# genjax-dev/genjax

Measured on AMD Instinct MI355X. Metric: particles/sec (particle-steps/s), bootstrap SMC sweep, linear-Gaussian SSM T=100, higher is better.
Workload: dtype f32; 1 GPU; BASELINE config 2: linear-Gaussian state-space (T=100), bootstrap SMC, systematic resampling every step; particles_per_gpu=1000000, particles_total=1000000, T=100, resampler=systematic, graph=True, key=314159

## Files before the change

### genjax_amd/_lib.py

```python
from __future__ import annotations

import ctypes
import os
from ctypes import (POINTER, Structure, c_char_p, c_float, c_int, c_int32, c_int64,
                    c_size_t, c_uint32, c_uint64, c_void_p)

import torch

GMX_MAX_IN = 64
GMX_MAX_OUT = 64
GMX_MAX_TAB = 8
GMX_MAX_UNI = 64

ABI_VERSION = 8
ANC_TAG_SHIFT = 24
ANC_INDEX_MASK = (1 << ANC_TAG_SHIFT) - 1
ANC_TAG_MAX = 255
KEY_NONE, KEY_ARRAY, KEY_SPLIT, KEY_ROWSPLIT, KEY_BCAST = 0, 1, 2, 3, 4
RESAMPLE_SYSTEMATIC, RESAMPLE_STRATIFIED, RESAMPLE_MULTINOMIAL, RESAMPLE_MULTINOMIAL_TILED = 0, 1, 2, 3
RESAMPLE_MULTINOMIAL_SORTED = 4


class ResampleIn(Structure):
    _fields_ = [
# ... 54 lines not shown
    _fields_ = [
        ("in_d", c_void_p * GMX_MAX_IN),
        ("out_d", c_void_p * GMX_MAX_OUT),
        ("tab_d", c_void_p * GMX_MAX_TAB),
        ("uni", c_uint32 * GMX_MAX_UNI),
        ("ancestors_d", c_void_p),
        ("key_mode", c_int32),
        ("key0", c_uint32),
        ("key1", c_uint32),
        ("keys_d", c_void_p),
        ("key_inner", c_int64),
        ("index_offset", c_int64),
        ("red_out_d", c_void_p),
        ("tile_agg_d", c_void_p),
        ("tile_shift", c_int32),
        ("reserved_", c_int32),
        ("step_stride", c_int64),
        ("rs", ResampleIn),
        ("sh", ShardIn),
        ("peer", Peer),
    ]


class GenmiError(RuntimeError):
    pass


_LIB_DIR = os.path.join(os.path.dirname(os.path.abspath(__file__)), "lib")
LIB_PATH = os.environ.get("GENMI_LIB") or os.path.join(_LIB_DIR, "libgenmi_hip.so")


class Backend:

    def __init__(self, cdll, device: torch.device, uses_streams: bool):
        self.c = cdll
        self.device = device
        self.uses_streams = uses_streams
        self._proto()

    def _proto(self):
        c = self.c
        c.gmx_run_args_bytes.restype = c_size_t
        if int(c.gmx_run_args_bytes()) != ctypes.sizeof(RunArgs):
            raise GenmiError(f"gmx_run_args is {c.gmx_run_args_bytes()} bytes in the library and {ctypes.sizeof(RunArgs)} in "
                             "this binding (genjax_amd/_lib.py): rebuild both from one include/genmi.h")
        c.gmx_version.restype = c_int
        c.gmx_last_error.restype = c_char_p
        c.gmx_threefry2x32_host.argtypes = [c_uint32, c_uint32, c_uint32, c_uint32, POINTER(c_uint32)]
        c.gmx_threefry2x32_host.restype = None
        c.gmx_split.argtypes = [POINTER(c_uint32), c_int64, c_int64, c_void_p, c_void_p]
        c.gmx_split_rows.argtypes = [c_void_p, c_int64, c_int64, c_void_p, c_void_p]
        c.gmx_fold_in.argtypes = [c_void_p, c_uint32, c_int64, c_void_p, c_void_p]
        c.gmx_random_bits.argtypes = [c_void_p, c_int64, c_int64, c_void_p, c_void_p]
        c.gmx_program_create.argtypes = [POINTER(c_uint32), c_size_t, POINTER(c_void_p)]
        c.gmx_program_destroy.argtypes = [c_void_p]
        c.gmx_program_specialize.argtypes = [c_void_p]
        c.gmx_program_is_specialized.argtypes = [c_void_p]
        c.gmx_program_code_hash.argtypes = [c_void_p]
        c.gmx_program_code_hash.restype = c_uint64
        c.gmx_program_despecialize.argtypes = [c_void_p, ctypes.c_char_p]
        c.gmx_jit_rejected_count.argtypes = []
        c.gmx_jit_rejected_count.restype = c_int64
        c.gmx_program_grid.argtypes = [c_void_p, c_int64]
        c.gmx_program_grid.restype = c_int64
        c.gmx_program_run.argtypes = [c_void_p, c_int64, POINTER(RunArgs), c_void_p]
        c.gmx_program_writes_tile_stats.argtypes = [c_void_p]
        c.gmx_program_set_background.argtypes = [c_void_p, c_uint32]
        c.gmx_program_set_fuse_resample.argtypes = [c_void_p]
        c.gmx_program_set_fuse_resample_loop.argtypes = [c_void_p]
        c.gmx_program_fuses_resample.argtypes = [c_void_p]
        c.gmx_program_set_fuse_shard_step.argtypes = [c_void_p]
        c.gmx_program_fuses_shard_step.argtypes = [c_void_p]
        c.gmx_program_resident_particles.argtypes = [c_void_p]
        c.gmx_program_resident_particles.restype = c_int64
        c.gmx_logsumexp_workspace.argtypes = [c_int64, c_int64]
        c.gmx_logsumexp_workspace.restype = c_size_t
        c.gmx_logsumexp.argtypes = [c_void_p, c_int64, c_int64, c_void_p, c_void_p, c_void_p, c_void_p]
        c.gmx_sum_rows_inorder.argtypes = [c_void_p, c_int64, c_int64, c_int64, c_int64, c_void_p, c_void_p]
        c.gmx_sum_rows_workspace.argtypes = [c_int64, c_int64]
        c.gmx_sum_rows_workspace.restype = c_size_t
        c.gmx_sum_rows.argtypes = [c_void_p, c_int64, c_int64, c_void_p, c_void_p, c_void_p]
        c.gmx_reduce_max.argtypes = [c_void_p, c_int64, c_void_p, c_void_p]
        c.gmx_weight_cdf_workspace.argtypes = [c_int64]
        c.gmx_weight_cdf_workspace.restype = c_size_t
        c.gmx_weight_cdf.argtypes = [c_void_p, c_int64, c_int, c_void_p, c_int64, c_void_p, c_void_p,
                                     c_void_p, c_void_p, c_void_p]
        c.gmx_ancestors.argtypes = [c_int, POINTER(c_uint32), c_void_p, c_int64, c_uint64, c_void_p,
                                    c_int64, c_int64, c_int64, c_void_p, c_void_p]
        c.gmx_multinomial_workspace.argtypes = [c_int64]
        c.gmx_multinomial_workspace.restype = c_size_t
        c.gmx_multinomial.argtypes = [POINTER(c_uint32), c_void_p, c_int64, c_void_p, c_int64, c_void_p, c_void_p, c_void_p]
        c.gmx_resample_workspace.argtypes = [c_int64]
        c.gmx_resample_workspace.restype = c_size_t
        c.gmx_resample.argtypes = [c_int, POINTER(c_uint32), c_void_p, c_int64, c_int, c_void_p, c_int64, c_void_p,
                                   c_void_p, c_void_p, c_void_p, c_void_p]
        c.gmx_tile_stats.argtypes = [c_void_p, c_int64, c_int, c_void_p, c_void_p, c_void_p]
        c.gmx_resample_tiles.argtypes = [c_int, POINTER(c_uint32), c_void_p, c_int64, c_int, c_void_p, c_void_p, c_void_p,
                                         c_void_p, c_void_p, c_void_p]
        c.gmx_multinomial_tiled_workspace.argtypes = [c_int64]
        c.gmx_multinomial_tiled_workspace.restype = c_size_t
        c.gmx_multinomial_tiled.argtypes = [POINTER(c_uint32), c_void_p, c_int64, c_int, c_void_p, c_void_p, c_void_p,
                                            c_void_p, c_void_p, c_void_p, c_void_p, c_int, c_void_p]
        c.gmx_slot_uniforms.argtypes = [c_void_p, c_int, c_int64, c_void_p, c_int, c_void_p]
        c.gmx_resample_tiles_u.argtypes = [c_int, POINTER(c_uint32), c_void_p, c_int64, c_int, c_void_p, c_void_p, c_void_p,
                                           c_void_p, c_void_p, c_void_p, c_void_p]
        c.gmx_sorted_uniforms_words.argtypes = [c_int64]
# ... 135 lines not shown
```

### genjax_amd/csrc/gmx_kernels.hip

```cpp
#include <hip/hip_runtime.h>
#include <hip/hiprtc.h>
#include <stdio.h>
#include <stdlib.h>
#include <string.h>
#include <sys/stat.h>
#include <unistd.h>

#include <new>
#include <atomic>
#include <string>
#include <vector>

#include "gmx_block.h"
#include "gmx_vm.h"
#include "gmx_resample.h"
#include "gmx_peer.h"
#include "gmx_sorted.h"
#include "gmx_offspring.h"
#include "gmx_shard_fill.h"

#define GMX_HIP(call)                                                        \
  do {                                                                       \
    hipError_t _e = (call);                                                  \
    if (_e != hipSuccess) return gmx_fail("%s (hip error %lld)", hipGetErrorString(_e), (long long)_e); \
// ... 756 lines not shown
  gmx_key k; k.k0 = kk.x; k.k1 = kk.y;
  gmx_key o = gmx_fold_in(k, data);
  reinterpret_cast<uint2*>(out)[i] = make_uint2(o.k0, o.k1);
}
__global__ void __launch_bounds__(GMX_BLOCK)
k_random_bits(const uint32_t* __restrict__ keys, int64_t n, int64_t m, uint32_t* __restrict__ out) {
  int64_t t = (int64_t)blockIdx.x * GMX_BLOCK + threadIdx.x;
  if (t >= n * m) return;
  int64_t i = t / m, j = t - i * m;
  uint2 kk = reinterpret_cast<const uint2*>(keys)[i];
  gmx_key k; k.k0 = kk.x; k.k1 = kk.y;
  out[t] = gmx_bits32(k, (uint64_t)j);
}

static inline dim3 grid_for(int64_t n) { return dim3((unsigned)((n + GMX_BLOCK - 1) / GMX_BLOCK)); }

extern "C" int gmx_split(const uint32_t key[2], int64_t n, int64_t index_offset,
                         uint32_t* out_keys_d, gmx_stream stream) {
  if (!key || (n > 0 && !out_keys_d)) return gmx_fail("gmx_split: null argument%s");
  if (n <= 0) return 0;
  hipLaunchKernelGGL(k_split, grid_for(n), dim3(GMX_BLOCK), 0, (hipStream_t)stream, key[0], key[1],
                     n, index_offset, out_keys_d);
  GMX_HIP(hipGetLastError());
  return 0;
}
extern "C" int gmx_split_rows(const uint32_t* keys_d, int64_t rows, int64_t inner,
                              uint32_t* out_keys_d, gmx_stream stream) {
  if (rows <= 0 || inner <= 0) return 0;
  if (!keys_d || !out_keys_d) return gmx_fail("gmx_split_rows: null argument%s");
  hipLaunchKernelGGL(k_split_rows, grid_for(rows * inner), dim3(GMX_BLOCK), 0, (hipStream_t)stream,
                     keys_d, rows, inner, out_keys_d);
  GMX_HIP(hipGetLastError());
  return 0;
}
extern "C" int gmx_fold_in(const uint32_t* keys_d, uint32_t data, int64_t n, uint32_t* out_d,
                           gmx_stream stream) {
  if (n <= 0) return 0;
  if (!keys_d || !out_d) return gmx_fail("gmx_fold_in: null argument%s");
  hipLaunchKernelGGL(k_fold_in, grid_for(n), dim3(GMX_BLOCK), 0, (hipStream_t)stream, keys_d, data, n,
                     out_d);
  GMX_HIP(hipGetLastError());
  return 0;
}
extern "C" int gmx_random_bits(const uint32_t* keys_d, int64_t n, int64_t m, uint32_t* out_d,
                               gmx_stream stream) {
  if (n <= 0 || m <= 0) return 0;
  if (!keys_d || !out_d) return gmx_fail("gmx_random_bits: null argument%s");
  hipLaunchKernelGGL(k_random_bits, grid_for(n * m), dim3(GMX_BLOCK), 0, (hipStream_t)stream, keys_d,
                     n, m, out_d);
  GMX_HIP(hipGetLastError());
  return 0;
}

#define LSE_ITEMS 16
#define LSE_TILE (GMX_BLOCK * LSE_ITEMS)
static_assert(LSE_TILE == GMX_LSE_TILE, "the row reductions' workspaces (gmx_sizes.h) are per tile of LSE_TILE columns");

__device__ __forceinline__ bool lse_finite(float m) { return m > -gmx_inf() && m < gmx_inf(); }
__device__ __forceinline__ float lse_nan_only(float x) { return x != x ? x : 0.0f; }

__global__ void __launch_bounds__(GMX_BLOCK)
k_lse_tiles(const float* __restrict__ lw, int64_t cols, int64_t tiles_per_row,
            float* __restrict__ partials) {
  __shared__ float lds4[4];
  int64_t row = blockIdx.y, tile = blockIdx.x;
  const float* x = lw + row * cols;
  int64_t base = tile * LSE_TILE;
  float v[LSE_ITEMS];
  float m = -gmx_inf();
#pragma unroll
  for (int k = 0; k < LSE_ITEMS; ++k) {
    int64_t j = base + (int64_t)k * GMX_BLOCK + threadIdx.x;
    v[k] = (j < cols) ? x[j] : -gmx_inf();
    m = gmx_rmax(m, v[k]);
  }
  m = block_max(m, lds4);
  float s = 0.0f;
  if (lse_finite(m)) {
#pragma unroll
    for (int k = 0; k < LSE_ITEMS; ++k) s += gmx_expf(v[k] - m);
  } else {
#pragma unroll
    for (int k = 0; k < LSE_ITEMS; ++k) s += lse_nan_only(v[k]);
  }
  s = block_sum(s, lds4);
  if (threadIdx.x == 0) {
    float* p = partials + 2 * (row * tiles_per_row + tile);
    p[0] = m; p[1] = s;
  }
}
__global__ void __launch_bounds__(GMX_BLOCK)
k_lse_final(const float* __restrict__ partials, int64_t n_part, float* __restrict__ out,
            float* __restrict__ out_max) {
  __shared__ float lds4[4];
  int64_t row = blockIdx.x;
  const float* p = partials + 2 * row * n_part;
  float m = -gmx_inf();
  for (int64_t j = threadIdx.x; j < n_part; j += GMX_BLOCK) m = gmx_rmax(m, p[2 * j]);
  m = block_max(m, lds4);
  float s = 0.0f;
  if (lse_finite(m))
    for (int64_t j = threadIdx.x; j < n_part; j += GMX_BLOCK)
      s += p[2 * j + 1] * gmx_expf(p[2 * j] - m);
  else
    for (int64_t j = threadIdx.x; j < n_part; j += GMX_BLOCK) s += lse_nan_only(p[2 * j + 1]);
  s = block_sum(s, lds4);
// ... 2630 lines not shown
```

### genjax_amd/csrc/gmx_math.h

```cpp
#pragma once
#if !defined(__HIPCC_RTC__)
#include <stdint.h>
#else
#include "genmi.h"
#endif

#if defined(__HIPCC__)
#define GMX_HD __host__ __device__ __forceinline__
#define GMX_HDM __host__ __device__ __forceinline__
#else
#define GMX_HD static inline
#define GMX_HDM inline
#endif

#define GMX_INF_BITS 0x7f800000u
#define GMX_NAN_BITS 0x7fc00000u

GMX_HD float gmx_u2f(uint32_t u) {
  union { uint32_t u; float f; } c; c.u = u; return c.f;
}
GMX_HD uint32_t gmx_f2u(float f) {
  union { uint32_t u; float f; } c; c.f = f; return c.u;
}
GMX_HD float gmx_fma(float a, float b, float c) { return __builtin_fmaf(a, b, c); }
// ... 57 lines not shown
  return nan ? x : y;
}

GMX_HD float gmx_expf_nonpos(float x) {
  const float lo = -87.33654022216797f;
  float xc = x < lo ? lo : x;
  float kf = __builtin_rintf(xc * 1.44269502162933349609375f);
  float r = gmx_fma(kf, -0.693359375f, xc);
  r = gmx_fma(kf, 2.12194440e-4f, r);
  float p = 1.9875691500e-4f;
  p = gmx_fma(p, r, 1.3981999507e-3f);
  p = gmx_fma(p, r, 8.3334519073e-3f);
  p = gmx_fma(p, r, 4.1665795894e-2f);
  p = gmx_fma(p, r, 1.6666665459e-1f);
  p = gmx_fma(p, r, 5.0000001201e-1f);
  float r2 = r * r;
  p = gmx_fma(p, r2, r);
  p = p + 1.0f;
  int k = gmx_isnan(x) ? 0 : (int)kf;
  int k1 = k >> 1;
  int k2 = k - k1;
  float y = (p * gmx_pow2i(k1)) * gmx_pow2i(k2);
  y = y < 1.17549435e-38f ? 0.0f : y;
  return x < lo ? 0.0f : y;
}

GMX_HD uint32_t gmx_exp_fixed_packed(float d, int shift) {
  const float lo = -87.33654022216797f;
  float dc = d > lo ? d : lo;
  dc = dc < 100.0f ? dc : 100.0f;
  const float kf = __builtin_rintf(dc * 1.44269502162933349609375f);
  float r = gmx_fma(kf, -0.693359375f, dc);
  r = gmx_fma(kf, 2.12194440e-4f, r);
  float p = 1.9875691500e-4f;
  p = gmx_fma(p, r, 1.3981999507e-3f);
  p = gmx_fma(p, r, 8.3334519073e-3f);
  p = gmx_fma(p, r, 4.1665795894e-2f);
  p = gmx_fma(p, r, 1.6666665459e-1f);
  p = gmx_fma(p, r, 5.0000001201e-1f);
  const float r2 = r * r;
  p = gmx_fma(p, r2, r);
  p = p + 1.0f;
  const uint32_t pb = gmx_f2u(p);
  uint32_t m = (pb & 0x007fffffu) | 0x00800000u;
  int32_t amt = 189 - (int32_t)(pb >> 23) - (int32_t)kf - shift;
  m = amt < 0 ? 0u : m;
  amt = amt > 63 ? 63 : amt;
  amt = amt < 0 ? 0 : amt;
  return m | ((uint32_t)amt << 24);
}
GMX_HD uint64_t gmx_fixed_unpack(uint32_t pk) { return ((uint64_t)(pk & 0x00ffffffu) << 39) >> (pk >> 24); }
GMX_HD uint64_t gmx_exp_fixed(float d, int shift) { return gmx_fixed_unpack(gmx_exp_fixed_packed(d, shift)); }

GMX_HD float gmx_logf(float x) {
  const uint32_t ux = gmx_f2u(x);
  const int den = ux < 0x00800000u;
  const float xs = den ? x * 8388608.0f : x;
  const uint32_t us = gmx_f2u(xs);
  int e = (den ? -23 : 0) + (int)(us >> 23) - 126;
  const float m = gmx_u2f((us & 0x007fffffu) | 0x3f000000u);
  const int low = m < 0.707106781186547524f;
  e -= low;
  const float f = low ? (m + m) - 1.0f : m - 1.0f;
  float z = f * f;
  float p = 7.0376836292e-2f;
  p = gmx_fma(p, f, -1.1514610310e-1f);
  p = gmx_fma(p, f, 1.1676998740e-1f);
  p = gmx_fma(p, f, -1.2420140846e-1f);
  p = gmx_fma(p, f, 1.4249322787e-1f);
  p = gmx_fma(p, f, -1.6668057665e-1f);
  p = gmx_fma(p, f, 2.0000714765e-1f);
  p = gmx_fma(p, f, -2.4999993993e-1f);
  p = gmx_fma(p, f, 3.3333331174e-1f);
  float y = (p * f) * z;
  float ef = (float)e;
  y = gmx_fma(ef, -2.12194440e-4f, y);
  y = gmx_fma(-0.5f, z, y);
  float r = f + y;
  r = gmx_fma(ef, 0.693359375f, r);
  r = (ux == GMX_INF_BITS) ? x : r;
  r = (ux >> 31) ? gmx_nan() : r;
  r = (ux == 0u || ux == 0x80000000u) ? -gmx_inf() : r;
  return gmx_isnan(x) ? x : r;
}

GMX_HD float gmx_log1pf(float x) {
  float u = 1.0f + x;
  float l = gmx_logf(u);
  float d = u - 1.0f;
  float r = l * (x / d);
  r = (gmx_f2u(u) == GMX_INF_BITS) ? u : r;
  r = (u == 1.0f) ? x : r;
  return gmx_isnan(x) ? x : r;
}

GMX_HD float gmx_sqrtf(float x) { return __builtin_sqrtf(x); }

GMX_HD float gmx_softplusf(float x) {
  float ax = gmx_fabs(x);
  float t = gmx_log1pf(gmx_expf(-ax));
  return (x > 0.0f ? x : 0.0f) + t;
}

GMX_HD float gmx_sigmoidf(float x) {
  if (x >= 0.0f) {
    float e = gmx_expf(-x);
    return 1.0f / (1.0f + e);
  }
  float e = gmx_expf(x);
  return e / (1.0f + e);
}

GMX_HD float gmx_tanhf(float x) {
  float ax = gmx_fabs(x);
  if (ax < 1e-4f) return x;
  float e = gmx_expf(-2.0f * ax);
  float t = (1.0f - e) / (1.0f + e);
  return (gmx_f2u(x) >> 31) ? -t : t;
}

GMX_HD float gmx_neg_log1m_sq(float x) {
  const float t = -(x * x);
  const float u = 1.0f + t;
  const uint32_t us = gmx_f2u(u);
  int e = (int)(us >> 23) - 126;
  const float m = gmx_u2f((us & 0x007fffffu) | 0x3f000000u);
  const int low = m < 0.707106781186547524f;
  e -= low;
  const float f = low ? (m + m) - 1.0f : m - 1.0f;
  float z = f * f;
  float p = 7.0376836292e-2f;
  p = gmx_fma(p, f, -1.1514610310e-1f);
  p = gmx_fma(p, f, 1.1676998740e-1f);
  p = gmx_fma(p, f, -1.2420140846e-1f);
  p = gmx_fma(p, f, 1.4249322787e-1f);
  p = gmx_fma(p, f, -1.6668057665e-1f);
  p = gmx_fma(p, f, 2.0000714765e-1f);
  p = gmx_fma(p, f, -2.4999993993e-1f);
  p = gmx_fma(p, f, 3.3333331174e-1f);
  float y = (p * f) * z;
  float ef = (float)e;
  y = gmx_fma(ef, -2.12194440e-4f, y);
  y = gmx_fma(-0.5f, z, y);
  float l = f + y;
  l = gmx_fma(ef, 0.693359375f, l);
  l = (us == 0u) ? -gmx_inf() : l;
  const float d = u - 1.0f;
  float r = l * (t / d);
  r = (u == 1.0f) ? t : r;
  return -r;
}

GMX_HD float gmx_erfinv_central(float w) {
  w = w - 2.5f;
  float p = 2.81022636e-08f;
  p = gmx_fma(p, w, 3.43273939e-07f);
  p = gmx_fma(p, w, -3.5233877e-06f);
  p = gmx_fma(p, w, -4.39150654e-06f);
  p = gmx_fma(p, w, 0.00021858087f);
  p = gmx_fma(p, w, -0.00125372503f);
  p = gmx_fma(p, w, -0.00417768164f);
  p = gmx_fma(p, w, 0.246640727f);
  p = gmx_fma(p, w, 1.50140941f);
  return p;
}
GMX_HD float gmx_erfinv_tail(float w) {
  w = gmx_sqrtf(w) - 3.0f;
  float p = -0.000200214257f;
  p = gmx_fma(p, w, 0.000100950558f);
  p = gmx_fma(p, w, 0.00134934322f);
  p = gmx_fma(p, w, -0.00367342844f);
  p = gmx_fma(p, w, 0.00573950773f);
  p = gmx_fma(p, w, -0.0076224613f);
  p = gmx_fma(p, w, 0.00943887047f);
  p = gmx_fma(p, w, 1.00167406f);
  p = gmx_fma(p, w, 2.83297682f);
  return p;
}
GMX_HD float gmx_erfinvf_from_w(float x, float w) {
  float p;
  if (w < 5.0f) p = gmx_erfinv_central(w);
  else p = gmx_erfinv_tail(w);
  if (gmx_fabs(x) == 1.0f) return x * gmx_inf();
  return p * x;
}
GMX_HD float gmx_erfinvf(float x) { return gmx_erfinvf_from_w(x, -gmx_log1pf(-(x * x))); }
GMX_HD float gmx_erfinvf_unit(float x) { return gmx_erfinvf_from_w(x, gmx_neg_log1m_sq(x)); }

GMX_HD float gmx_lgammaf(float x) {
  if (gmx_isnan(x)) return x;
  if (x <= 0.0f) return gmx_inf();
  if (gmx_f2u(x) == GMX_INF_BITS) return x;
  float shift = 0.0f;
  if (x < 8.0f) {
    float prod = 1.0f;
    while (x < 8.0f) {
      prod = prod * x;
      x = x + 1.0f;
    }
    shift = gmx_logf(prod);
  }
// ... 63 lines not shown
```

### genjax_amd/csrc/gmx_offspring.h

```cpp
#pragma once
#include "gmx_block.h"
#include "gmx_resample.h"
#include "gmx_sorted.h"

#define CDF_VEC_OT 4
#ifndef RS_THREADS
#define RS_THREADS 256
#endif
#define RS_TILE (RS_THREADS * CDF_VEC_OT)
#define RS_MAX_TILES GMX_MAX_TILES
static_assert(RS_TILE == GMX_TILE && RS_THREADS == GMX_BLOCK, "resampling tiles are the CDF's definition tiles");
static_assert(RS_MAX_TILES % GMX_BLOCK == 0, "tile table shape");

#define GMX_ANC_TAG_SHIFT 24
#define GMX_ANC_INDEX_MASK 0xffffffu
#define GMX_ANC_TAG_MAX 255u
__device__ __forceinline__ void gmx_store_u32x4_sc1(uint32_t* p, uint32_t a, uint32_t b, uint32_t c, uint32_t d) {
  typedef uint32_t v4 __attribute__((ext_vector_type(4)));
  v4 v; v.x = a; v.y = b; v.z = c; v.w = d;
  asm volatile("s_nop 1\n\tglobal_store_dwordx4 %0, %1, off sc1\n\ts_nop 1" :: "v"(p), "v"(v) : "memory");
}
__device__ __forceinline__ void gmx_store_u32x8_sc1(uint32_t* base_uniform, uint32_t off, uint4 a, uint4 b) {
  typedef uint32_t v4 __attribute__((ext_vector_type(4)));
  v4 va, vb; va.x = a.x; va.y = a.y; va.z = a.z; va.w = a.w; vb.x = b.x; vb.y = b.y; vb.z = b.z; vb.w = b.w;
// ... 4 lines not shown
  __hip_atomic_store(p, a, __ATOMIC_RELAXED, __HIP_MEMORY_SCOPE_AGENT);
}

typedef uint32_t rs_u32x4_a4 __attribute__((ext_vector_type(4), aligned(4)));
typedef uint32_t sorted_u32x2_a4 __attribute__((ext_vector_type(2), aligned(4)));
struct sorted_ctx {
  const uint32_t* slow; const uint32_t* guide; const uint64_t* toff;
  uint64_t stot, gmax; uint32_t sh, mask; double ratio;
};
__device__ __forceinline__ sorted_ctx sorted_ctx_of(const uint32_t* table, int64_t n, uint64_t total, uint64_t stot, uint32_t sh) {
  const gmx_sorted_layout L = gmx_sorted_layout_of(n);
  sorted_ctx X;
  X.slow = table; X.guide = table + L.off_guide;
  X.toff = reinterpret_cast<const uint64_t*>(table + L.off_toff);
  X.stot = stot;
  X.sh = sh;
  X.mask = (1u << X.sh) - 1u;
  X.gmax = X.stot >> X.sh;
  X.ratio = (double)X.stot / (double)(total ? total : 1ull);
  return X;
}
__device__ __forceinline__ int64_t sorted_below_exact(const sorted_ctx& X, uint64_t c, uint64_t total, int64_t j, int64_t n) {
  const u128 R = mul64(c, X.stot);
  j = j < 0 ? 0 : (j > n ? n : j);
  auto below = [&](int64_t k) {
    const uint64_t off = X.toff[k >> 10];
    const uint64_t S = off + (uint64_t)(uint32_t)(X.slow[k] - (uint32_t)off);
    return gt128(R, mul64(S, total));
  };
  while (j > 0 && !below(j - 1)) --j;
  while (j < n && below(j)) ++j;
  return j;
}

#define RS_TPB 1
#define GMX_KEEP_BRANCH asm volatile("")
__device__ __forceinline__ uint64_t rs_zext_here(uint32_t o) { asm volatile("" : "+v"(o)); return (uint64_t)o; }
#define RS_BLOCK (GMX_BLOCK * RS_TPB)
#define RS_WAVES (RS_BLOCK / GMX_WAVE)
static_assert(RS_MAX_TILES % RS_BLOCK == 0, "tile table shape");
#define RS_FILL_SLOTS 2048
template <int kind, int PER, bool TAGGED>
__device__ __forceinline__ void
gmx_offspring_tile_body(uint32_t k0, uint32_t k1, uint32_t u0_host, const float* __restrict__ lw,
                        const float* __restrict__ tmax, const uint64_t* __restrict__ agg, int64_t n, int n_tiles, float scale,
                        float* __restrict__ max_out, uint64_t* __restrict__ total_out, int32_t* __restrict__ anc,
                        const uint32_t* __restrict__ uslot, uint32_t tag,
                        int tile0 = -1, uint64_t a_prefix = 0ull, uint64_t a_total = 0ull, uint64_t a_mk = 0ull) {
  const int blk = tile0 >= 0 ? tile0 : (int)blockIdx.x;
  const uint32_t tagw = TAGGED ? (tag << GMX_ANC_TAG_SHIFT) : 0u;
  __shared__ uint64_t s_below[RS_WAVES], s_all[RS_WAVES], s_scan[RS_WAVES], s_g[RS_TPB];
  __shared__ float s_max[RS_WAVES];
  const int lane = threadIdx.x & 63, wave = threadIdx.x >> 6;
  const int grp = RS_TPB > 1 ? (int)(threadIdx.x >> 8) : 0, ltid = threadIdx.x & (GMX_BLOCK - 1);
  const int first_tile = blk * RS_TPB;
  const int my_tile = first_tile + grp;
  const bool tile_ok = my_tile < n_tiles;
  const int tile_c = tile_ok ? my_tile : n_tiles - 1;
  const int64_t i0 = (int64_t)tile_c * RS_TILE + (int64_t)ltid * CDF_VEC_OT;
  float x[CDF_VEC_OT];
  const bool full_tile = (int64_t)(tile_c + 1) * RS_TILE <= n;
  if (full_tile) {
    float4 v = *reinterpret_cast<const float4*>(lw + i0);
    x[0] = v.x; x[1] = v.y; x[2] = v.z; x[3] = v.w;
  } else {
#pragma unroll
    for (int c = 0; c < CDF_VEC_OT; ++c) {
      const int64_t ic = i0 + c < n ? i0 + c : n - 1;
      const float xv = lw[ic];
      x[c] = (i0 + c < n) ? xv : -gmx_inf();
    }
  }
  constexpr bool PREF = (PER == 0);
  constexpr int PERN = PREF ? 1 : PER;
  static_assert(PER >= 0 && PER * RS_BLOCK <= RS_MAX_TILES, "rows of the tile table per thread");
  static_assert(!PREF || RS_TPB == 1, "the prefix form works on one tile per block");
  uint64_t ta[PERN];
  float tm[PERN];
  const uint32_t tid4 = threadIdx.x * 4u;
  uint64_t pf_prefix = 0, pf_total = 0, pf_mk = 0;
  if (PREF) {
    if (agg) { pf_prefix = agg[tile_c]; pf_total = agg[n_tiles]; pf_mk = agg[n_tiles + 1]; }
    else { pf_prefix = a_prefix; pf_total = a_total; pf_mk = a_mk; }
  } else {
#pragma unroll
    for (int r = 0; r < PERN; ++r) {
      ta[r] = 0ull; tm[r] = -gmx_inf();
      if (r * RS_BLOCK < n_tiles) {
        if ((r + 1) * RS_BLOCK <= n_tiles) {
          GMX_KEEP_BRANCH;
          uint32_t r0 = (uint32_t)(r * RS_BLOCK);
          asm volatile("" : "+s"(r0));
          ta[r] = *reinterpret_cast<const uint64_t*>(reinterpret_cast<const char*>(agg + r0) + rs_zext_here(tid4 * 2u));
          tm[r] = *reinterpret_cast<const float*>(reinterpret_cast<const char*>(tmax + r0) + rs_zext_here(tid4));
        } else {
          const int t = r * RS_BLOCK + (int)threadIdx.x;
          const int tc = t < n_tiles ? t : n_tiles - 1;
          ta[r] = agg[tc];
          tm[r] = tmax[tc];
        }
      }
    }
  }
  const float tmax_mine = tmax[tile_c];
  uint64_t sx_stot = 0; uint32_t sx_sh = 0;
  if constexpr (kind == GMX_RESAMPLE_MULTINOMIAL_SORTED) {
    const gmx_sorted_layout L = gmx_sorted_layout_of(n);
    sx_stot = reinterpret_cast<const uint64_t*>(uslot + L.off_toff)[L.tiles];
    sx_sh = uslot[L.off_sh];
  }
  __builtin_amdgcn_sched_barrier(0);
  if (!PREF) {
#pragma unroll
    for (int r = 0; r < PERN; ++r) {
      if (r * RS_BLOCK < n_tiles && (r + 1) * RS_BLOCK > n_tiles) {
        GMX_KEEP_BRANCH;
        const int t = r * RS_BLOCK + (int)threadIdx.x;
        ta[r] = (t < n_tiles) ? ta[r] : 0ull;
        tm[r] = (t < n_tiles) ? tm[r] : -gmx_inf();
      }
    }
  }
  const int32_t k_b = gmx_tile_exp(tmax_mine);
  const float ref_b = gmx_tile_ref(k_b);
  float M = -gmx_inf();
  if (PREF) {
    M = gmx_u2f((uint32_t)pf_mk);
  } else {
#pragma unroll
    for (int r = 0; r < PERN; ++r)
      if (r * RS_BLOCK < n_tiles) M = gmx_rmax(M, tm[r]);
    M = wave_max(M);
  }
  uint64_t q[CDF_VEC_OT];
  uint64_t run = 0;
#pragma unroll
  for (int c = 0; c < CDF_VEC_OT; ++c) q[c] = weight_fixed(x[c], ref_b, scale);
  if (!(tile_ok && full_tile)) {
    GMX_KEEP_BRANCH;
#pragma unroll
    for (int c = 0; c < CDF_VEC_OT; ++c) q[c] = (tile_ok && i0 + c < n) ? q[c] : 0ull;
  }
#pragma unroll
  for (int c = 0; c < CDF_VEC_OT; ++c) {
    run += q[c];
    q[c] = run;
  }
  const uint64_t inc = wave_scan_u64(run);
  if (!PREF && lane == 0) s_max[wave] = M;
  if (lane == 63) s_scan[wave] = inc;
  __syncthreads();
  if (!PREF) {
    M = s_max[0];
#pragma unroll
    for (int w = 1; w < RS_WAVES; ++w) M = gmx_rmax(M, s_max[w]);
  }
  uint64_t wave_off = 0;
#pragma unroll
  for (int w = 0; w < 4; ++w) wave_off += (w < (wave & 3)) ? s_scan[4 * grp + w] : 0ull;
  const uint64_t loc = wave_off + (inc - run);
  const int32_t K = PREF ? (int32_t)(uint32_t)(pf_mk >> 32) : gmx_tile_exp(M);
  uint64_t prefix = 0, total = 0;
  if (PREF) {
    prefix = pf_prefix; total = pf_total;
  } else {
    uint64_t below = 0, all = 0;
#pragma unroll
    for (int r = 0; r < PERN; ++r) {
      if (r * RS_BLOCK < n_tiles) {
        const int t = r * RS_BLOCK + (int)threadIdx.x;
        const uint64_t G = gmx_tile_scale(ta[r], gmx_tile_exp(tm[r]), K);
        all += G;
        if ((r + 1) * RS_BLOCK <= first_tile) { GMX_KEEP_BRANCH; below += G; }
        else if (r * RS_BLOCK < first_tile) { GMX_KEEP_BRANCH; below += (t < first_tile) ? G : 0ull; }
        if constexpr (RS_TPB > 1)
          if (t >= first_tile && t < first_tile + RS_TPB) s_g[t - first_tile] = G;
      }
    }
    wave_sum2_u64(below, all);
    if (lane == 0) { s_below[wave] = below; s_all[wave] = all; }
    __syncthreads();
#pragma unroll
    for (int w = 0; w < RS_WAVES; ++w) { prefix += s_below[w]; total += s_all[w]; }
    if constexpr (RS_TPB > 1) {
#pragma unroll
      for (int j = 0; j < RS_TPB; ++j) prefix += (j < grp) ? s_g[j] : 0ull;
    }
  }
  if (blk == 0 && threadIdx.x == 0) { *total_out = total; *max_out = M; }
  if (!tile_ok) return;
  gmx_key key; key.k0 = k0; key.k1 = k1;
  if (total == 0) {
#pragma unroll
    for (int c = 0; c < CDF_VEC_OT; ++c)
      if (i0 + c < n) {
        if (TAGGED) gmx_store_u32_sc1(reinterpret_cast<uint32_t*>(anc) + (i0 + c), (uint32_t)(n - 1) | tagw);
        else anc[i0 + c] = (int32_t)(n - 1);
      }
    return;
  }
  const double n_over_total = (double)n / (double)total;
  const double eps = (double)n * 0x1p-44 + 0x1p-40;
  const int32_t n32 = (int32_t)n;
  uint64_t cv[CDF_VEC_OT + 1];
  cv[0] = prefix + gmx_tile_scale(loc, k_b, K);
#pragma unroll
  for (int c = 0; c < CDF_VEC_OT; ++c) cv[c + 1] = prefix + gmx_tile_scale(loc + q[c], k_b, K);
  if (!full_tile) {
    GMX_KEEP_BRANCH;
#pragma unroll
    for (int c = 0; c < CDF_VEC_OT; ++c) cv[c + 1] = (i0 + c < n) ? cv[c + 1] : total;
  }
// ... 89 lines not shown
  if (__any(near)) {
    const uint64_t D = (uint64_t)n << 23;
    int32_t fixed0 = e[0];
#pragma unroll 1
    for (int c = 0; c <= CDF_VEC_OT; ++c) {
      if (near_bits & (1u << c)) {
        const uint64_t cc = c == 0 ? cv[0] : c == 1 ? cv[1] : c == 2 ? cv[2] : c == 3 ? cv[3] : cv[4];
        const int32_t j0 = c == 0 ? e[0] : c == 1 ? e[1] : c == 2 ? e[2] : c == 3 ? e[3] : e[4];
        int32_t j;
        if constexpr (SORTED) j = (int32_t)sorted_below_exact(SX, cc, total, (int64_t)j0, n);
        else j = (int32_t)slots_below_exact(kind, key, (uint64_t)u0_host, cc, D, total, (int64_t)j0, n);
        if (c == 0) fixed0 = j; else if (c == 1) e[1] = j; else if (c == 2) e[2] = j; else if (c == 3) e[3] = j; else e[4] = j;
      }
    }
    const uint32_t up = wave_shr1_u32((uint32_t)e[CDF_VEC_OT], (uint32_t)fixed0);
    e[0] = (lane == 0) ? fixed0 : (int32_t)up;
  }
  __shared__ int32_t s_edge[RS_WAVES];
  if (lane == 63) s_edge[wave] = e[CDF_VEC_OT];
  const int32_t e4 = e[4];
  const uint32_t src0t = (uint32_t)(int32_t)i0 | tagw;
  static_assert(RS_TPB == 1, "the LDS fill works on one tile per block");
  __shared__ __attribute__((aligned(16))) uint32_t s_mark[RS_FILL_SLOTS];
  __shared__ int32_t s_rng[2];
  __shared__ uint32_t s_carry[RS_WAVES];
  if (threadIdx.x == 0) s_rng[0] = e[0];
  if (threadIdx.x == RS_BLOCK - 1) s_rng[1] = e4;
  reinterpret_cast<uint4*>(s_mark)[threadIdx.x] = make_uint4(0u, 0u, 0u, 0u);
  reinterpret_cast<uint4*>(s_mark)[threadIdx.x + RS_BLOCK] = make_uint4(0u, 0u, 0u, 0u);
  __syncthreads();
  if (lane == 0 && wave > 0) e[0] = s_edge[wave - 1];
  const int32_t T0 = __builtin_amdgcn_readfirstlane(s_rng[0]), T1 = __builtin_amdgcn_readfirstlane(s_rng[1]);
  for (int32_t base = T0; base < T1; base += RS_FILL_SLOTS) {
    if (base != T0) {
      reinterpret_cast<uint4*>(s_mark)[threadIdx.x] = make_uint4(0u, 0u, 0u, 0u);
      reinterpret_cast<uint4*>(s_mark)[threadIdx.x + RS_BLOCK] = make_uint4(0u, 0u, 0u, 0u);
      __syncthreads();
    }
#pragma unroll
    for (int c = 0; c < CDF_VEC_OT; ++c) {
      const int32_t lo = e[c] > base ? e[c] : base;
      if (e[c + 1] > lo && lo - base < RS_FILL_SLOTS) s_mark[lo - base] = src0t + (uint32_t)c;
    }
    __syncthreads();
    uint4 a = reinterpret_cast<const uint4*>(s_mark)[2 * threadIdx.x];
    uint4 b = reinterpret_cast<const uint4*>(s_mark)[2 * threadIdx.x + 1];
    a.y = a.y > a.x ? a.y : a.x; a.z = a.z > a.y ? a.z : a.y; a.w = a.w > a.z ? a.w : a.z;
    b.x = b.x > a.w ? b.x : a.w; b.y = b.y > b.x ? b.y : b.x; b.z = b.z > b.y ? b.z : b.y; b.w = b.w > b.z ? b.w : b.z;
    const uint32_t incl = gmx_wave_umax_scan(b.w);
    uint32_t carry = wave_shr1_u32(incl, 0u);
    if (lane == 63) s_carry[wave] = incl;
    __syncthreads();
#pragma unroll
    for (int w = 0; w < RS_WAVES - 1; ++w) { const uint32_t v = s_carry[w]; carry = (w < wave && v > carry) ? v : carry; }
    a.x = a.x > carry ? a.x : carry; a.y = a.y > carry ? a.y : carry; a.z = a.z > carry ? a.z : carry; a.w = a.w > carry ? a.w : carry;
    b.x = b.x > carry ? b.x : carry; b.y = b.y > carry ? b.y : carry; b.z = b.z > carry ? b.z : carry; b.w = b.w > carry ? b.w : carry;
    const int32_t j = base + 8 * (int32_t)threadIdx.x;
    if (j + 8 <= T1) {
      rs_u32x4_a4 va, vb;
      va.x = a.x; va.y = a.y; va.z = a.z; va.w = a.w; vb.x = b.x; vb.y = b.y; vb.z = b.z; vb.w = b.w;
      if (TAGGED) {
        gmx_store_u32x8_sc1(reinterpret_cast<uint32_t*>(anc) + base, 32u * threadIdx.x, a, b);
      } else {
        *reinterpret_cast<rs_u32x4_a4*>(anc + j) = va;
        *reinterpret_cast<rs_u32x4_a4*>(anc + j + 4) = vb;
      }
    } else {
      if (j + 0 < T1) { if (TAGGED) gmx_store_u32_sc1(reinterpret_cast<uint32_t*>(anc) + j + 0, a.x); else anc[j + 0] = (int32_t)a.x; }
      if (j + 1 < T1) { if (TAGGED) gmx_store_u32_sc1(reinterpret_cast<uint32_t*>(anc) + j + 1, a.y); else anc[j + 1] = (int32_t)a.y; }
      if (j + 2 < T1) { if (TAGGED) gmx_store_u32_sc1(reinterpret_cast<uint32_t*>(anc) + j + 2, a.z); else anc[j + 2] = (int32_t)a.z; }
      if (j + 3 < T1) { if (TAGGED) gmx_store_u32_sc1(reinterpret_cast<uint32_t*>(anc) + j + 3, a.w); else anc[j + 3] = (int32_t)a.w; }
      if (j + 4 < T1) { if (TAGGED) gmx_store_u32_sc1(reinterpret_cast<uint32_t*>(anc) + j + 4, b.x); else anc[j + 4] = (int32_t)b.x; }
      if (j + 5 < T1) { if (TAGGED) gmx_store_u32_sc1(reinterpret_cast<uint32_t*>(anc) + j + 5, b.y); else anc[j + 5] = (int32_t)b.y; }
      if (j + 6 < T1) { if (TAGGED) gmx_store_u32_sc1(reinterpret_cast<uint32_t*>(anc) + j + 6, b.z); else anc[j + 6] = (int32_t)b.z; }
      if (j + 7 < T1) { if (TAGGED) gmx_store_u32_sc1(reinterpret_cast<uint32_t*>(anc) + j + 7, b.w); else anc[j + 7] = (int32_t)b.w; }
    }
  }
}



__device__ __forceinline__ void
gmx_tile_table_pass(const float* __restrict__ tmax, const uint64_t* __restrict__ agg, int n_tiles, int blk, int G, int C,
                    uint64_t* __restrict__ s_pf , uint64_t& total, uint64_t& mk) {
  __shared__ float s_tm[RS_WAVES];
  __shared__ uint64_t s_acc[RS_WAVES][2];
  const int lane = threadIdx.x & 63, wave = threadIdx.x >> 6;
  float M = -gmx_inf();
  for (int t = (int)threadIdx.x; t < n_tiles; t += RS_BLOCK) M = gmx_rmax(M, tmax[t]);
  M = wave_max(M);
  if (lane == 0) s_tm[wave] = M;
  __syncthreads();
  M = s_tm[0];
#pragma unroll
  for (int w = 1; w < RS_WAVES; ++w) M = gmx_rmax(M, s_tm[w]);
  const int32_t K = gmx_tile_exp(M);
  uint64_t running = 0;
#pragma clang loop unroll(disable)
  for (int c = 0; c < C; ++c) {
    const int lo = c * G, hi = (lo + G < n_tiles) ? lo + G : n_tiles, mine = lo + blk;
    uint64_t tot = 0, part = 0;
    for (int tb = lo; tb < hi; tb += RS_BLOCK) {
      const int t = tb + (int)threadIdx.x;
      if (t < hi) {
        const uint64_t g_ = gmx_tile_scale(agg[t], gmx_tile_exp(tmax[t]), K);
        tot += g_;
        if (tb + RS_BLOCK <= mine) { GMX_KEEP_BRANCH; part += g_; }
// ... 17 lines not shown
```

### genjax_amd/csrc/gmx_rng.h

```cpp
#pragma once
#include "gmx_math.h"

struct gmx_key { uint32_t k0, k1; };

GMX_HD uint32_t gmx_rotl(uint32_t x, int r) { return (x << r) | (x >> (32 - r)); }

#define GMX_TF_ROUND(r)            \
  x0 += x1;                        \
  x1 = gmx_rotl(x1, r);            \
  x1 ^= x0;

GMX_HD void gmx_threefry2x32(uint32_t k0, uint32_t k1, uint32_t c0, uint32_t c1,
                              uint32_t* o0, uint32_t* o1) {
  uint32_t ks0 = k0, ks1 = k1, ks2 = k0 ^ k1 ^ 0x1BD11BDAu;
  uint32_t x0 = c0 + ks0, x1 = c1 + ks1;
  GMX_TF_ROUND(13) GMX_TF_ROUND(15) GMX_TF_ROUND(26) GMX_TF_ROUND(6)
  x0 += ks1; x1 += ks2 + 1u;
  GMX_TF_ROUND(17) GMX_TF_ROUND(29) GMX_TF_ROUND(16) GMX_TF_ROUND(24)
  x0 += ks2; x1 += ks0 + 2u;
  GMX_TF_ROUND(13) GMX_TF_ROUND(15) GMX_TF_ROUND(26) GMX_TF_ROUND(6)
  x0 += ks0; x1 += ks1 + 3u;
  GMX_TF_ROUND(17) GMX_TF_ROUND(29) GMX_TF_ROUND(16) GMX_TF_ROUND(24)
  x0 += ks1; x1 += ks2 + 4u;
  GMX_TF_ROUND(13) GMX_TF_ROUND(15) GMX_TF_ROUND(26) GMX_TF_ROUND(6)
  x0 += ks2; x1 += ks0 + 5u;
  *o0 = x0; *o1 = x1;
}

GMX_HD gmx_key gmx_split_child(gmx_key k, uint64_t i) {
  gmx_key o;
  gmx_threefry2x32(k.k0, k.k1, (uint32_t)(i >> 32), (uint32_t)i, &o.k0, &o.k1);
  return o;
}
GMX_HD gmx_key gmx_fold_in(gmx_key k, uint32_t d) {
  gmx_key o;
  gmx_threefry2x32(k.k0, k.k1, 0u, d, &o.k0, &o.k1);
  return o;
}
GMX_HD uint32_t gmx_bits32(gmx_key k, uint64_t j) {
  uint32_t a, b;
  gmx_threefry2x32(k.k0, k.k1, (uint32_t)(j >> 32), (uint32_t)j, &a, &b);
  return a ^ b;
}

GMX_HD float gmx_bits_to_unit(uint32_t bits) {
  return gmx_u2f((bits >> 9) | 0x3f800000u) - 1.0f;
}
GMX_HD float gmx_uniform_from_bits(uint32_t bits, float lo, float hi) {
  float u = gmx_bits_to_unit(bits);
  float v = u * (hi - lo);
  v = v + lo;
  return v > lo ? v : lo;
}
GMX_HD float gmx_std_normal_from_bits(uint32_t bits) {
  const float lo = -0.99999994f;
  float u = gmx_uniform_from_bits(bits, lo, 1.0f);
  return 1.41421354f * gmx_erfinvf_unit(u);
}
GMX_HD float gmx_gumbel_from_bits(uint32_t bits) {
  const float tiny = 1.17549435e-38f;
  float u = gmx_uniform_from_bits(bits, tiny, 1.0f);
  return -gmx_logf(-gmx_logf(u));
}
```

### genjax_amd/csrc/gmx_vm.h

```cpp
#pragma once
#include "genmi.h"
#include "gmx_dist.h"
#include "gmx_program.h"

template <int N>
struct gmx_regs_vgpr {
#if defined(__HIPCC__)
  typedef uint32_t vec_t __attribute__((ext_vector_type(N)));
  vec_t v;
  GMX_HDM void init() { v = (vec_t)(0u); }
#else
  uint32_t v[N];
  GMX_HDM void init() { for (int k = 0; k < N; ++k) v[k] = 0u; }
#endif
  GMX_HDM uint32_t get(uint32_t i) const { return v[i]; }
  GMX_HDM void set(uint32_t i, uint32_t x) { v[i] = x; }
};

GMX_HD int64_t gmx_rowsplit_row(int64_t i, int64_t inner) {
#if defined(__HIP_DEVICE_COMPILE__)
  if (gridDim.y > 1) return (int64_t)blockIdx.y;
#endif
  return i / inner;
}
// ... 192 lines not shown
        }
        break;
    }
    const uint32_t dreg = (op == OP_STOUT) ? 0u : dst;
    if (wr >= 1) R.set(dreg, r0);
    if (wr == 2) R.set(dreg + 1u, r1);
  }
#undef SRC
#undef FSRC
#undef KEY
#undef ELEM
}

template <class Regs, bool FULL, int NI, class Ctx>
GMX_HD void gmx_vm_run(uint32_t n_instr_rt, int64_t i, bool active, const gmx_run_args& A, Ctx& ctx) {
  Regs R;
  R.init();
  uint32_t t = 0u, tf = 0u, heads = 0u, head3 = 0u;
  int depth = 0;
  for (uint32_t pc = 0; pc < n_instr_rt; ++pc) {
    gmx_rword w;
    ctx.fetch(pc, &w.a, &w.b);
    const uint32_t op = w.a & 0xffu;
    if (op == OP_LOOP) {
      if (depth == 0) { heads = pc; depth = 1; t = 0u; tf = 0u; }
      else if (depth == 1) { heads = (heads & 0xffffu) | (pc << 16); depth = 2; tf = tf * w.b; t = 0u; }
      else { head3 = pc; depth = 3; tf = tf * w.b; t = 0u; }
      continue;
    }
    if (op == OP_ENDLOOP) {
      gmx_rword h;
      const uint32_t hp = depth == 3 ? head3 : (depth == 2 ? (heads >> 16) : (heads & 0xffffu));
      ctx.fetch(hp, &h.a, &h.b);
      if (t + 1u < h.b) { ++t; ++tf; pc = hp; }
      else if (depth == 3) {
        gmx_rword h2;
        ctx.fetch(heads >> 16, &h2.a, &h2.b);
        depth = 2; tf = tf / h.b; t = tf % h2.b;
      }
      else if (depth == 2) { depth = 1; t = tf / h.b; tf = t; }
      else { depth = 0; t = 0u; tf = 0u; }
      continue;
    }
    gmx_vm_step<Regs, FULL, gmx_rword, Ctx>(R, w, i, active, A, ctx, t, tf);
  }
}

GMX_HD bool gmx_op_needs_full(uint32_t op) {
  return op == OP_POW || op == OP_SIN || op == OP_COS || op == OP_TANH || op == OP_SOFTPLUS ||
         op == OP_LGAMMA || op == OP_S_BETA || op == OP_S_CATSTEP || op == OP_L_BETA || op == OP_S_LOGGAMMA;
}

#if defined(__cplusplus) && !defined(__HIPCC__) && !defined(__HIPCC_RTC__)
#include "gmx_history.h"
#include "gmx_backward.h"
#include "gmx_resample_rows.h"
#endif
```

### include/genmi.h

```cpp
#ifndef GENMI_H
#define GENMI_H

#if defined(__HIPCC_RTC__)
typedef __UINT8_TYPE__ uint8_t;
typedef __UINT16_TYPE__ uint16_t;
typedef __UINT32_TYPE__ uint32_t;
typedef __UINT64_TYPE__ uint64_t;
typedef __INT32_TYPE__ int32_t;
typedef __INT64_TYPE__ int64_t;
typedef __SIZE_TYPE__ size_t;
typedef __UINTPTR_TYPE__ uintptr_t;
#else
#include <stddef.h>
#include <stdint.h>
#endif

#ifdef __cplusplus
extern "C" {
#endif

#define GMX_ABI_VERSION 8

typedef void* gmx_stream;
typedef struct gmx_program gmx_program;

int gmx_version(void);
size_t gmx_run_args_bytes(void);
const char* gmx_last_error(void);


void gmx_threefry2x32_host(uint32_t k0, uint32_t k1, uint32_t c0, uint32_t c1,
                           uint32_t out[2]);

int gmx_split(const uint32_t key[2], int64_t n, int64_t index_offset,
              uint32_t* out_keys_d , gmx_stream stream);
int gmx_split_rows(const uint32_t* keys_d , int64_t rows,
                   int64_t inner, uint32_t* out_keys_d ,
                   gmx_stream stream);
int gmx_fold_in(const uint32_t* keys_d , uint32_t data, int64_t n,
                uint32_t* out_d , gmx_stream stream);
int gmx_random_bits(const uint32_t* keys_d , int64_t n, int64_t m,
                    uint32_t* out_d , gmx_stream stream);


#define GMX_MAX_IN 64
#define GMX_MAX_OUT 64
#define GMX_MAX_TAB 8
#define GMX_MAX_UNI 64

enum {
  GMX_KEY_NONE = 0,
  GMX_KEY_ARRAY = 1,
  GMX_KEY_SPLIT = 2,
  GMX_KEY_ROWSPLIT = 3,
  GMX_KEY_BCAST = 4
};

typedef struct gmx_resample_in {
  const float* lw_d;
  const float* tile_max_d;
  const uint64_t* tile_agg_d;
  float* max_out_d;
  uint64_t* total_out_d;
  uint64_t* status_d;
  int32_t shift;
  uint32_t tag;
  uint32_t key0, key1;
  uint32_t u0;
  uint32_t reserved_;
} gmx_resample_in;

#define GMX_PEER_MAX_LEAVES 32
typedef struct gmx_peer {
  void* const* land_d;
  const uint32_t* tag_base_d;
  uint64_t* status_d;
  int32_t rank, world;
  int32_t step;
  int32_t tiles;
  int64_t capacity;
  int32_t leaves;
  int32_t reserved_;
} gmx_peer;

typedef struct gmx_shard_in {
  const float* lw_d;
  const void* stats_own_d;
  int64_t* plan_d;
  uint64_t* total_out_d;
  float* max_out_d;
  uint64_t* status_d;
  int32_t shift;
  uint32_t tag;
  uint32_t key0, key1;
  uint32_t u0;
// ... 233 lines not shown
```

Baseline: 75.79 billion particle-steps/s.

## Add std-normal-from-bits entry point and tweak log/div/uniform math helpers

Adds a new exported std-normal-from-bits kernel, with a host fallback and a ctypes binding. It also rewrites the log mantissa/exponent split into a branchless bias trick and replaces a float division with a reciprocal plus Newton refinement. The uniform clamp in the normal sampler now uses fmaxf, and the wave index in the offspring kernel is made wave-uniform with readfirstlane. These are mostly small arithmetic trims mixed with new API surface. The new log split and division may change rounding slightly.

```diff
diff --git a/genjax_amd/_lib.py b/genjax_amd/_lib.py
--- a/genjax_amd/_lib.py
+++ b/genjax_amd/_lib.py
@@ -130,6 +130,7 @@
         c.gmx_split_rows.argtypes = [c_void_p, c_int64, c_int64, c_void_p, c_void_p]
         c.gmx_fold_in.argtypes = [c_void_p, c_uint32, c_int64, c_void_p, c_void_p]
         c.gmx_random_bits.argtypes = [c_void_p, c_int64, c_int64, c_void_p, c_void_p]
+        c.gmx_std_normal_from_bits.argtypes = [c_void_p, c_int64, c_void_p, c_void_p]
         c.gmx_program_create.argtypes = [POINTER(c_uint32), c_size_t, POINTER(c_void_p)]
         c.gmx_program_destroy.argtypes = [c_void_p]
         c.gmx_program_specialize.argtypes = [c_void_p]
diff --git a/genjax_amd/csrc/gmx_draw_tail.h b/genjax_amd/csrc/gmx_draw_tail.h
--- /dev/null
+++ b/genjax_amd/csrc/gmx_draw_tail.h
@@ -0,0 +1,12 @@
+#pragma once
+#if defined(__cplusplus) && !defined(__HIPCC__) && !defined(__HIPCC_RTC__)
+#include "genmi.h"
+#include "gmx_rng.h"
+#include "gmx_sizes.h"
+extern "C" __attribute__((used)) inline int gmx_std_normal_from_bits(const uint32_t* bits_d, int64_t n, float* out_d, gmx_stream) {
+  if (n <= 0) return 0;
+  if (!bits_d || !out_d) return gmx_fail("gmx_std_normal_from_bits: null argument%s");
+  for (int64_t i = 0; i < n; ++i) out_d[i] = gmx_std_normal_from_bits(bits_d[i]);
+  return 0;
+}
+#endif
diff --git a/genjax_amd/csrc/gmx_kernels.hip b/genjax_amd/csrc/gmx_kernels.hip
--- a/genjax_amd/csrc/gmx_kernels.hip
+++ b/genjax_amd/csrc/gmx_kernels.hip
@@ -832,6 +832,21 @@
   return 0;
 }
 
+__global__ void __launch_bounds__(GMX_BLOCK)
+k_std_normal_from_bits(const uint32_t* __restrict__ bits, int64_t n, float* __restrict__ out) {
+  const int64_t stride = (int64_t)gridDim.x * GMX_BLOCK;
+  for (int64_t i = (int64_t)blockIdx.x * GMX_BLOCK + threadIdx.x; i < n; i += stride) out[i] = gmx_std_normal_from_bits(bits[i]);
+}
+extern "C" int gmx_std_normal_from_bits(const uint32_t* bits_d, int64_t n, float* out_d, gmx_stream stream) {
+  if (n <= 0) return 0;
+  if (!bits_d || !out_d) return gmx_fail("gmx_std_normal_from_bits: null argument%s");
+  const int64_t blocks = (n + GMX_BLOCK - 1) / GMX_BLOCK;
+  hipLaunchKernelGGL(k_std_normal_from_bits, dim3((unsigned)(blocks < 8192 ? blocks : 8192)), dim3(GMX_BLOCK), 0,
+                     (hipStream_t)stream, bits_d, n, out_d);
+  GMX_HIP(hipGetLastError());
+  return 0;
+}
+
 #define LSE_ITEMS 16
 #define LSE_TILE (GMX_BLOCK * LSE_ITEMS)
 static_assert(LSE_TILE == GMX_LSE_TILE, "the row reductions' workspaces (gmx_sizes.h) are per tile of LSE_TILE columns");
diff --git a/genjax_amd/csrc/gmx_math.h b/genjax_amd/csrc/gmx_math.h
--- a/genjax_amd/csrc/gmx_math.h
+++ b/genjax_amd/csrc/gmx_math.h
@@ -133,16 +133,20 @@
 GMX_HD uint64_t gmx_fixed_unpack(uint32_t pk) { return ((uint64_t)(pk & 0x00ffffffu) << 39) >> (pk >> 24); }
 GMX_HD uint64_t gmx_exp_fixed(float d, int shift) { return gmx_fixed_unpack(gmx_exp_fixed_packed(d, shift)); }
 
+GMX_HD void gmx_log_split(uint32_t us, int* e, float* f) {
+  const uint32_t ix = us + (0x3f800000u - 0x3f3504f3u);
+  *e = (int)(ix >> 23) - 127;
+  *f = gmx_u2f((ix & 0x007fffffu) + 0x3f3504f3u) - 1.0f;
+}
+
 GMX_HD float gmx_logf(float x) {
   const uint32_t ux = gmx_f2u(x);
   const int den = ux < 0x00800000u;
   const float xs = den ? x * 8388608.0f : x;
   const uint32_t us = gmx_f2u(xs);
-  int e = (den ? -23 : 0) + (int)(us >> 23) - 126;
-  const float m = gmx_u2f((us & 0x007fffffu) | 0x3f000000u);
-  const int low = m < 0.707106781186547524f;
-  e -= low;
-  const float f = low ? (m + m) - 1.0f : m - 1.0f;
+  int e; float f;
+  gmx_log_split(us, &e, &f);
+  e += den ? -23 : 0;
   float z = f * f;
   float p = 7.0376836292e-2f;
   p = gmx_fma(p, f, -1.1514610310e-1f);
@@ -200,15 +204,27 @@
   return (gmx_f2u(x) >> 31) ? -t : t;
 }
 
+#if defined(__HIP_DEVICE_COMPILE__)
+GMX_HD float gmx_div_near(float t, float d) {
+  float rc = __builtin_amdgcn_rcpf(d);
+  const float er = gmx_fma(-d, rc, 1.0f);
+  rc = gmx_fma(er, rc, rc);
+  float q = t * rc;
+  float rem = gmx_fma(-d, q, t);
+  q = gmx_fma(rem, rc, q);
+  rem = gmx_fma(-d, q, t);
+  return gmx_fma(rem, rc, q);
+}
+#else
+GMX_HD float gmx_div_near(float t, float d) { return t / d; }
+#endif
+
 GMX_HD float gmx_neg_log1m_sq(float x) {
   const float t = -(x * x);
   const float u = 1.0f + t;
   const uint32_t us = gmx_f2u(u);
-  int e = (int)(us >> 23) - 126;
-  const float m = gmx_u2f((us & 0x007fffffu) | 0x3f000000u);
-  const int low = m < 0.707106781186547524f;
-  e -= low;
-  const float f = low ? (m + m) - 1.0f : m - 1.0f;
+  int e; float f;
+  gmx_log_split(us, &e, &f);
   float z = f * f;
   float p = 7.0376836292e-2f;
   p = gmx_fma(p, f, -1.1514610310e-1f);
@@ -227,7 +243,7 @@
   l = gmx_fma(ef, 0.693359375f, l);
   l = (us == 0u) ? -gmx_inf() : l;
   const float d = u - 1.0f;
-  float r = l * (t / d);
+  float r = l * gmx_div_near(t, d);
   r = (u == 1.0f) ? t : r;
   return -r;
 }
diff --git a/genjax_amd/csrc/gmx_offspring.h b/genjax_amd/csrc/gmx_offspring.h
--- a/genjax_amd/csrc/gmx_offspring.h
+++ b/genjax_amd/csrc/gmx_offspring.h
@@ -80,6 +80,7 @@
   __shared__ uint64_t s_below[RS_WAVES], s_all[RS_WAVES], s_scan[RS_WAVES], s_g[RS_TPB];
   __shared__ float s_max[RS_WAVES];
   const int lane = threadIdx.x & 63, wave = threadIdx.x >> 6;
+  const int wave_s = __builtin_amdgcn_readfirstlane(wave);
   const int grp = RS_TPB > 1 ? (int)(threadIdx.x >> 8) : 0, ltid = threadIdx.x & (GMX_BLOCK - 1);
   const int first_tile = blk * RS_TPB;
   const int my_tile = first_tile + grp;
@@ -185,7 +186,7 @@
   }
   uint64_t wave_off = 0;
 #pragma unroll
-  for (int w = 0; w < 4; ++w) wave_off += (w < (wave & 3)) ? s_scan[4 * grp + w] : 0ull;
+  for (int w = 0; w < 4; ++w) wave_off += (w < (wave_s & 3)) ? s_scan[4 * grp + w] : 0ull;
   const uint64_t loc = wave_off + (inc - run);
   const int32_t K = PREF ? (int32_t)(uint32_t)(pf_mk >> 32) : gmx_tile_exp(M);
   uint64_t prefix = 0, total = 0;
@@ -381,7 +382,7 @@
     if (lane == 63) s_carry[wave] = incl;
     __syncthreads();
 #pragma unroll
-    for (int w = 0; w < RS_WAVES - 1; ++w) { const uint32_t v = s_carry[w]; carry = (w < wave && v > carry) ? v : carry; }
+    for (int w = 0; w < RS_WAVES - 1; ++w) { const uint32_t v = s_carry[w]; carry = (w < wave_s && v > carry) ? v : carry; }
     a.x = a.x > carry ? a.x : carry; a.y = a.y > carry ? a.y : carry; a.z = a.z > carry ? a.z : carry; a.w = a.w > carry ? a.w : carry;
     b.x = b.x > carry ? b.x : carry; b.y = b.y > carry ? b.y : carry; b.z = b.z > carry ? b.z : carry; b.w = b.w > carry ? b.w : carry;
     const int32_t j = base + 8 * (int32_t)threadIdx.x;
diff --git a/genjax_amd/csrc/gmx_rng.h b/genjax_amd/csrc/gmx_rng.h
--- a/genjax_amd/csrc/gmx_rng.h
+++ b/genjax_amd/csrc/gmx_rng.h
@@ -54,7 +54,9 @@
 }
 GMX_HD float gmx_std_normal_from_bits(uint32_t bits) {
   const float lo = -0.99999994f;
-  float u = gmx_uniform_from_bits(bits, lo, 1.0f);
+  float v = gmx_bits_to_unit(bits) * (1.0f - lo);
+  v = v + lo;
+  const float u = __builtin_fmaxf(v, lo);
   return 1.41421354f * gmx_erfinvf_unit(u);
 }
 GMX_HD float gmx_gumbel_from_bits(uint32_t bits) {
diff --git a/genjax_amd/csrc/gmx_vm.h b/genjax_amd/csrc/gmx_vm.h
--- a/genjax_amd/csrc/gmx_vm.h
+++ b/genjax_amd/csrc/gmx_vm.h
@@ -268,6 +268,7 @@
 }
 
 #if defined(__cplusplus) && !defined(__HIPCC__) && !defined(__HIPCC_RTC__)
+#include "gmx_draw_tail.h"
 #include "gmx_history.h"
 #include "gmx_backward.h"
 #include "gmx_resample_rows.h"
diff --git a/include/genmi.h b/include/genmi.h
--- a/include/genmi.h
+++ b/include/genmi.h
@@ -41,6 +41,8 @@
                 uint32_t* out_d , gmx_stream stream);
 int gmx_random_bits(const uint32_t* keys_d , int64_t n, int64_t m,
                     uint32_t* out_d , gmx_stream stream);
+int gmx_std_normal_from_bits(const uint32_t* bits_d , int64_t n, float* out_d ,
+                             gmx_stream stream);
 
 
 #define GMX_MAX_IN 64
```

Result: faster. 77.84 billion particle-steps/s (median of 6 runs) (+2.7%).
